# shadimsaleh/motion_detection

Hardware: AMD Instinct MI355X
Metric: Mpixels/s (flow+warp+diff) at 1080p & 4K; % HBM roofline, 1/2/4/8 GPU (higher is better)
Workload: dtype u8

## Files before the change

### motion_detection_amd/csrc/mdx_ctx.h

```cpp
#pragma once

#include "../../include/mdx.h"
#include "mdx_internal.h"

#include <algorithm>
#include <array>
#include <cstdarg>
#include <cstdio>
#include <initializer_list>
#include <string>
#include <utility>
#include <vector>

struct DevBuf {
    void* p = nullptr;
    size_t cap = 0;
    DevBuf() = default;
    DevBuf(DevBuf&& o) noexcept : p(std::exchange(o.p, nullptr)), cap(std::exchange(o.cap, 0)) {}
    DevBuf& operator=(DevBuf&& o) noexcept
    {
        std::swap(p, o.p), std::swap(cap, o.cap);
        return *this;
    }
    ~DevBuf() { reset(); }
// ... 33 lines not shown
    std::vector<hipStream_t> streams;
    std::vector<hipEvent_t> events;
    std::vector<void*> pinned;
    hipStream_t stream = nullptr;
    hipStream_t aux = nullptr;
    hipEvent_t lkev[mdx::kMaxLevels + 2] = {};
    hipStream_t iter2 = nullptr;
    hipEvent_t flowev[2] = {};
    hipEvent_t front_ev = nullptr;
    hipEvent_t pyr_free[2] = {};
    hipEvent_t lvl_done[mdx::kMaxLevels] = {};
    hipEvent_t redo_ev[mdx::kMaxLevels] = {};
    mdx::LkLaunch lk;
    int pyr_half = 0;
    hipEvent_t input_ev = nullptr;
    uint8_t* last_pyr1 = nullptr;
    uint8_t* last_pyr2 = nullptr;
    uint8_t* band_pyr1 = nullptr;
    uint8_t* band_pyr2 = nullptr;
    int band_half = 0;
    const uint8_t* band_img1 = nullptr;
    int band_built[2] = {0, 0};
    int band_stride = 0, band_fmt = 0;
    DevBuf errw;
    int* err_host = nullptr;
    int* tcnt_host = nullptr;
    long long lk_fallback[3] = {0, 0, 0};
    mdx_params prm{};
    int max_w = 0, max_h = 0, max_batch = 0;
    DevBuf pyr1, pyr2, der, fits;
    DevBuf in1, in2, np, st, vec, mask, H, Hext, num;
    DevBuf bnp, bst;
    DevBuf cls, Abuf, ctab;
    DevBuf dbg;
    DevBuf lkcnt;
    DevBuf csum;
    DevBuf tin, tcur, tnp, tst, ttraj, tnum, tflag;
    DevBuf straj, sdata, sq, scnt, scols, sres, sout, sbest;
    DevBuf clpts, clbest, clroot;
    std::vector<int32_t> cl_host;
    DevBuf vcpts, vcroot, vcrows, vcq;
    std::vector<double> vc_host;
    std::vector<float> vc_pts;
    std::vector<int32_t> vc_idx;
    DevBuf hlin, hlout;
    std::vector<int32_t> hl_in, hl_out;
    std::vector<int32_t> hl_idx;
    DevBuf olin, olmag, olout;
    std::vector<double> ol_host;
    std::vector<uint8_t> ol_flags;
    DevBuf rgscr;
    DevBuf rgin, rgout;
    DevBuf rhscr;
    DevBuf rhout;
    DevBuf ring_pyr, ring_der, rin;
    DevBuf rfull;
    DevBuf hsrc, hdst;
    DevBuf wscr;
    mdx::WarpLaunch last_warp;
    DevBuf rsc;
    std::vector<int> ring_order;
    int ring_cap = 0, ring_w = 0, ring_h = 0, ring_ml = -1;
    std::array<size_t, 4> lk_scratch_key{{0, 0, 0, 0}};
    std::array<int, 6> plan_key{{-1, -1, -1, -1, -1, -1}};
    int band_w = 0, band_h = 0;
    mdx::ClassPlan plan{};
// ... 118 lines not shown
```

### motion_detection_amd/csrc/mdx_internal.h

```cpp
#pragma once

#include <hip/hip_runtime.h>
#include <math.h>
#include <stdint.h>

#include <algorithm>

#include "mdx.h"
#include "mdx_plan.h"

namespace mdx {

static_assert(sizeof(float4) == kFloat4Bytes, "lk_scratch sizes the A sums by it");
constexpr int kLkDbgStampOff = kMaxLevels * 64 + 64;
constexpr int kLkDbgWaves = 16384;

inline uint8_t* level0_core(uint8_t* slab, const Geometry& g) { return slab + g.lv[0].img_off + g.lv[0].core(); }

struct PairFit {
    double H[9];
    double Hinv[9];
    int num_vectors;
    int fit_status;
    int src_y0, src_y1;
// ... 74 lines not shown
    int* num;
    double mvs;
    float* htraj;
    int* htlen;
    float* hstart;
    double* hvec;
};
hipError_t launch_lk_chain(hipStream_t s, const LkArgs& a, const TrajChain& t, int ppw);
size_t subspace_basis_bytes(int n, int d, int precision);
hipError_t launch_subspace(hipStream_t s, const float* traj, int N, int T, int d, const int* cols, int nhyp,
                           double sigma, float* data, void* basis, int* counts, double* residuals,
                           uint8_t* is_outlier, int* best, int precision);
constexpr int kClB = 256;
hipError_t launch_cluster(hipStream_t s, const float* pts, int N, uint32_t slim, unsigned long long* best,
                          int32_t* root);
size_t vcluster_rows_bytes(int nA);
hipError_t launch_vcluster(hipStream_t s, const double* xyt, int nA, double slim, double athr, int abs_int,
                           uint32_t* rows, uint32_t* qscan, uint32_t* cand, int32_t* root);
hipError_t launch_outliers(hipStream_t s, int batch, int n, const double* dxy, double* ang, double* mag,
                           int include_zeros, uint8_t* flags, mdx_outlier_stats* stats, bool in_registers);
hipError_t launch_traj_init(hipStream_t s, int npts, int ny, int pixel_step, int nimg, float* cur, float* traj,
                            int* tlen, int* num, int* flag = nullptr);
hipError_t launch_traj_update(hipStream_t s, int npts, const float* next_pts, const uint8_t* status, float* cur,
                              float* traj, int* tlen, int nimg, int w, int h, int last, double min_vector_size,
                              double* vectors, float* start_pts, int* num);
struct LkLaunch {
    hipStream_t s = nullptr;
    hipStream_t aux = nullptr;
    hipStream_t s2 = nullptr;
    hipEvent_t* ev = nullptr;
    hipEvent_t* flow_ev = nullptr;
    hipEvent_t* redo_ev = nullptr;
    uint8_t* cls = nullptr;
    float4* Ab = nullptr;
    uint8_t* cert = nullptr;
    int* qctr = nullptr;
    int* done = nullptr;
    hipEvent_t* lvl_done = nullptr;
    hipEvent_t prev_ready = nullptr;
};
hipError_t launch_lk_v2(const LkLaunch& L, int batch, const LkArgs& a);
constexpr int kRansacMaxIters = 1024;
struct RansacArgs {
    int iters;
    double thresh;
    uint32_t seed;
    int* list;
    double* hyps;
    int* counts;
};
struct RansacScratch {
    size_t hyps, counts, bytes;
};
inline RansacScratch ransac_scratch(int batch, int npts, int iters)
{
    const size_t list_b = (size_t)batch * npts * sizeof(int), hyps_b = (size_t)batch * iters * 9 * sizeof(double),
                 counts_b = (size_t)batch * iters * sizeof(int);
    RansacScratch L;
    L.hyps = (list_b + 7) & ~(size_t)7;
    L.counts = L.hyps + hyps_b;
    L.bytes = list_b + hyps_b + counts_b + 256;
    return L;
}
inline size_t ransac_scratch_bytes(int batch, int npts, int iters) { return ransac_scratch(batch, npts, iters).bytes; }
inline RansacArgs ransac_args(void* base, int batch, int npts, const mdx_params& P)
{
// ... 108 lines not shown
```

### motion_detection_amd/csrc/mdx_lk.hip

```cpp
#include "mdx_dev.h"

#include <float.h>

#include <algorithm>
#include <atomic>
#include <cstdlib>
#include <type_traits>

namespace mdx {

typedef short s2 __attribute__((ext_vector_type(2)));
typedef float f2 __attribute__((ext_vector_type(2)));
typedef unsigned int v4u __attribute__((ext_vector_type(4)));
typedef unsigned int v3u __attribute__((ext_vector_type(3)));
struct LkRunRsrc {
    unsigned long long base;
    uint32_t bytes;

    __device__ __forceinline__ LkRunRsrc(const void* p, uint32_t n)
    {
        const unsigned long long b = (unsigned long long)(uintptr_t)p;
        const uint32_t lo = __builtin_amdgcn_readfirstlane((uint32_t)b);
        const uint32_t hi = __builtin_amdgcn_readfirstlane((uint32_t)(b >> 32)) & 0xffffu;
        base = ((unsigned long long)hi << 32) | lo;
// ... 86 lines not shown
__device__ __forceinline__ void lk_vmcnt()
{
    static_assert(N >= 0 && N < 16, "vmcnt field");
    __builtin_amdgcn_sched_barrier(0);
    __builtin_amdgcn_s_waitcnt(0x0F70 | N);
    __builtin_amdgcn_sched_barrier(0);
}

template <int B, int E, typename F>
__device__ __forceinline__ void static_for(F&& f)
{
    if constexpr (B < E) {
        f(std::integral_constant<int, B>{});
        static_for<B + 1, E>(f);
    }
}

__device__ __forceinline__ int xcd_remap(int b, int total)
{
    const int xcd = b & 7, q = total >> 3, r = total & 7;
    return (xcd < r ? xcd * (q + 1) : r * (q + 1) + (xcd - r) * q) + (b >> 3);
}

__device__ __forceinline__ void cls_store(uint4* o, const uint32_t (&dv)[4], const int (&cv)[4])
{
    typedef unsigned v4nt __attribute__((ext_vector_type(4)));
    const uint4 a = make_uint4(dv[0], (uint32_t)cv[0], dv[1], (uint32_t)cv[1]);
    const uint4 b = make_uint4(dv[2], (uint32_t)cv[2], dv[3], (uint32_t)cv[3]);
    __builtin_nontemporal_store(__builtin_bit_cast(v4nt, a), reinterpret_cast<v4nt*>(o));
    __builtin_nontemporal_store(__builtin_bit_cast(v4nt, b), reinterpret_cast<v4nt*>(o) + 1);
}

__global__ __launch_bounds__(256) void k_lk_class(const uint8_t* __restrict__ pyr1, const uint32_t* __restrict__ der,
                                                  uint8_t* __restrict__ cls_out, LkClassArgs a)
{
    const int level = a.level;
    const ClassLevel& C = a.plan.lv[level];
    const int nclass = C.nrx * C.nry;
    const int pair = blockIdx.z / nclass, cls = blockIdx.z % nclass;
    const int j = blockIdx.x * blockDim.x + threadIdx.x;
    const int v = C.vlo + blockIdx.y;
    if (4 * j >= a.g.lv[level].w + 2 * kPad || v >= C.UH) return;
    const Level L = a.g.lv[level];
    const float scale = (float)(1. / (1 << level));
    const int rx = residue_of(a.rlist, level, 0, cls % C.nrx), ry = residue_of(a.rlist, level, 1, cls / C.nrx);
    const float ppx = (float)rx * scale - 19.5f, ppy = (float)ry * scale - 19.5f;
    const float fa = ppx - floorf(ppx), fb = ppy - floorf(ppy);
    int w00, w01, w10, w11;
    lk_weights(fa, fb, w00, w01, w10, w11);
    const uint8_t* I = pyr1 + (long long)pair * a.g.img_bytes + L.img_off + L.core();
    const uint32_t* D = der + (long long)pair * a.g.der_words + L.der_off + L.core();
    const int y = v - kPad;
    const int p = L.pitch;
    uint8_t* base = cls_out + (long long)pair * a.plan.bytes_per_pair + C.off + (long long)cls * C.class_bytes;
    uint32_t dv[4] = {0, 0, 0, 0};
    int cv[4];
    const int x0 = 4 * j - kPad;
    if (y < L.h + kPad - 1 && x0 < L.w + kPad - 1) {
        const uint8_t* ip = I + (long long)y * p + x0;
        const uint32_t* dp = D + (long long)y * p + x0;
        uint32_t ib[2][2], dw[2][5];
#pragma unroll
        for (int r = 0; r < 2; r++) {
            const u2a4k bi = *reinterpret_cast<const u2a4k*>(ip + (long long)r * p);
            ib[r][0] = bi.x; ib[r][1] = bi.y;
            const uint4 d4 = *reinterpret_cast<const uint4*>(dp + (long long)r * p);
            dw[r][0] = d4.x; dw[r][1] = d4.y; dw[r][2] = d4.z; dw[r][3] = d4.w;
            dw[r][4] = dp[(long long)r * p + 4];
        }
        const s2 W0 = {(short)w00, (short)w01}, W1 = {(short)w10, (short)w11};
        static_for<0, 4>([&](auto qc) {
            constexpr int q = decltype(qc)::value;
            if (x0 + q >= L.w + kPad - 1) { cv[q] = lk_class_c(0); return; }
            int ival, ixv, iyv;
            lk_interp<q>(ib[0][0], ib[0][1], ib[1][0], ib[1][1], dw[0][q], dw[0][q + 1], dw[1][q], dw[1][q + 1], W0, W1,
                         ival, ixv, iyv);
            dv[q] = ((uint32_t)ixv & 0xffffu) | ((uint32_t)iyv << 16);
            cv[q] = lk_class_c(ival);
        });
    } else {
#pragma unroll
        for (int q = 0; q < 4; q++) cv[q] = lk_class_c(0);
    }
    uint4* o = reinterpret_cast<uint4*>(base) + ((long long)v * C.PW + 4 * j) / 2;
    cls_store(o, dv, cv);
}

__global__ __launch_bounds__(256) void k_lk_class_fused(const uint8_t* __restrict__ pyr1, uint8_t* __restrict__ cls_out,
                                                        LkClassArgs a)
{
    const int level = a.level;
    const ClassLevel& C = a.plan.lv[level];
    const int nclass = C.nrx * C.nry;
    const int pair = blockIdx.z;
    const int j = blockIdx.x * blockDim.x + threadIdx.x;
    const int v = C.vlo + blockIdx.y;
    if (4 * j >= a.g.lv[level].w + 2 * kPad || v >= C.UH) return;
    const Level L = a.g.lv[level];
    const float scale = (float)(1. / (1 << level));
    const uint8_t* I = pyr1 + (long long)pair * a.g.img_bytes + L.img_off + L.core();
    const int y = v - kPad;
    const int p = L.pitch;
    const int x0 = 4 * j - kPad;
    const bool inside = y < L.h + kPad - 1 && x0 < L.w + kPad - 1;
    uint32_t rw[4][3];
#pragma unroll
    for (int r = 0; r < 4; r++) {
        const int yy = y - 1 + r;
        const int ys = (yy < -kPad || yy >= L.h + kPad) ? y : yy;
        const u3a4k t = *reinterpret_cast<const u3a4k*>(I + (long long)ys * p + x0 - 4);
        rw[r][0] = t.x; rw[r][1] = t.y; rw[r][2] = t.z;
    }
    uint32_t dw[2][5];
#pragma unroll
    for (int r = 0; r < 2; r++) {
        const int yy = y + r;
#pragma unroll
        for (int c = 0; c < 5; c++) {
            const int x = x0 + c;
            const bool in = yy >= 0 && yy < L.h && x >= 0 && x < L.w;
            dw[r][c] = in ? scharr_word(rw[r], rw[r + 1], rw[r + 2], 4 + c) : 0u;
        }
    }
    for (int cls = 0; cls < nclass; cls++) {
        const int rx = residue_of(a.rlist, level, 0, cls % C.nrx), ry = residue_of(a.rlist, level, 1, cls / C.nrx);
        const float ppx = (float)rx * scale - 19.5f, ppy = (float)ry * scale - 19.5f;
        const float fa = ppx - floorf(ppx), fb = ppy - floorf(ppy);
        int w00, w01, w10, w11;
        lk_weights(fa, fb, w00, w01, w10, w11);
        uint32_t dv[4] = {0, 0, 0, 0};
        int cv[4] = {lk_class_c(0), lk_class_c(0), lk_class_c(0), lk_class_c(0)};
        if (inside) {
            const s2 W0 = {(short)w00, (short)w01}, W1 = {(short)w10, (short)w11};
            static_for<0, 4>([&](auto qc) {
                constexpr int q = decltype(qc)::value;
                if (x0 + q >= L.w + kPad - 1) return;
                int ival, ixv, iyv;
                lk_interp<q>(rw[1][1], rw[1][2], rw[2][1], rw[2][2], dw[0][q], dw[0][q + 1], dw[1][q], dw[1][q + 1], W0,
                             W1, ival, ixv, iyv);
                dv[q] = ((uint32_t)ixv & 0xffffu) | ((uint32_t)iyv << 16);
                cv[q] = lk_class_c(ival);
            });
        }
        uint8_t* base = cls_out + (long long)pair * a.plan.bytes_per_pair + C.off + (long long)cls * C.class_bytes;
        uint4* o = reinterpret_cast<uint4*>(base) + ((long long)v * C.PW + 4 * j) / 2;
        cls_store(o, dv, cv);
    }
}

template <int G, int UW>
struct LkShape {
    static constexpr int UWIDTH = UW;
    static constexpr int LPS = 4 * G;
    static constexpr int S = 64 / LPS;
    static constexpr int NP = (UW + 2 * LPS - 1) / (2 * LPS);
    static constexpr int BYTES = S * UW * 8;
    static constexpr int ND = (BYTES + 1023) / 1024;
    static_assert(UW % 2 == 0 && UW >= kWin, "union width");
};

struct GroupGeom {
    int gx, gy;
    bool valid;
    int ipx, ipy;
    int off;
    int v0;
    uint32_t ubase;
};

template <int G, int UW>
__device__ __forceinline__ GroupGeom group_geom(const LkArgs& a, const ClassLevel& C, int level, int g, int sl)
{
    GroupGeom r;
    const int16_t* xo = a.ord + C.ord_off;
    const int16_t* yo = xo + C.nxp;
    const bool has = g >= 0;
    const int gg = has ? g : 0;
    const int cg = gg / a.nyg, row = gg - cg * a.nyg;
    const int e0 = cg * G;
// ... 44 lines not shown
#pragma unroll
        for (int c = 0; c < Sh::ND; c++)
            if (1024 * c + 16 * lane >= Sh::BYTES) uoff[c] = 0x80000000u;
    }
    template <int B>
    __device__ __forceinline__ void dma(const uint32_t (&uoff)[Sh::ND])
    {
        lds_u32* I = ibuf<B>();
        const __amdgpu_buffer_rsrc_t r = crs.rsrc();
#pragma unroll
        for (int c = 0; c < Sh::ND; c++)
            __builtin_amdgcn_raw_ptr_buffer_load_lds(r, (lds_ptr)(I + 256 * c), 16, (int)uoff[c], 0, 0, 0);
        crs.advance(rowb);
    }
};

__device__ __forceinline__ float4 lk_A_result(f2 sd, float s12, bool ok, float min_eig)
{
    constexpr float FLT_SCALE = 1.f / (1 << 20);
    const float a11 = ((quad_bcast<0>(sd.x) + quad_bcast<1>(sd.x)) + quad_bcast<2>(sd.x)) + quad_bcast<3>(sd.x);
    const float a12 = ((quad_bcast<0>(s12) + quad_bcast<1>(s12)) + quad_bcast<2>(s12)) + quad_bcast<3>(s12);
    const float a22 = ((quad_bcast<0>(sd.y) + quad_bcast<1>(sd.y)) + quad_bcast<2>(sd.y)) + quad_bcast<3>(sd.y);
    const float A11 = a11 * FLT_SCALE, A12 = a12 * FLT_SCALE, A22 = a22 * FLT_SCALE;
    float Dinv = 0.f;
    if (ok) {
        const float D = A11 * A22 - A12 * A12;
        const float minEig = (A22 + A11 - __builtin_sqrtf((A11 - A22) * (A11 - A22) + 4.f * A12 * A12)) /
                             (float)(2 * kWin * kWin);
        if (!(minEig < min_eig || D < FLT_EPSILON)) Dinv = 1.f / D;
    }
    return make_float4(A11, A12, A22, Dinv);
}

constexpr float kLkCertMax = 2056.f;
static_assert(kLkCertMax * 8160.f < 16777216.f, "certified products are exact in float");
__device__ __forceinline__ float lk_mag_max(float m, f2 f)
{
    return __builtin_fmaxf(__builtin_fmaxf(m, __builtin_fabsf(f.x)), __builtin_fabsf(f.y));
}
__device__ __forceinline__ f2 lk_fma(f2 f, float fd, f2 acc) { return __builtin_elementwise_fma(f, f2{fd, fd}, acc); }
__device__ __forceinline__ uint8_t lk_cert_flag(float m)
{
    const float q = __builtin_fmaxf(__builtin_fmaxf(quad_bcast<0>(m), quad_bcast<1>(m)),
                                    __builtin_fmaxf(quad_bcast<2>(m), quad_bcast<3>(m)));
    return q <= kLkCertMax ? 1 : 0;
}

template <int G, int UW>
__global__ __launch_bounds__(64) void k_lk_A(LkArgs a, const uint8_t* __restrict__ cls, float4* __restrict__ Ab,
                                             uint8_t* __restrict__ cert, int* __restrict__ qctr, int level, int ngroups)
{
    using Sh = LkShape<G, UW>;
    constexpr int LPS = Sh::LPS, S = Sh::S, ND = Sh::ND;
    constexpr int NB = 3;
    __shared__ __attribute__((aligned(16))) uint32_t img0[ND * 256];
    __shared__ __attribute__((aligned(16))) uint32_t img1[ND * 256];
    __shared__ __attribute__((aligned(16))) uint32_t img2[ND * 256];

    const int lane = threadIdx.x, k = lane & 3, slot = lane / LPS, sl = lane % LPS;
    const int nw = gridDim.x;
    const int bid = xcd_remap(blockIdx.x + nw * blockIdx.y, nw * gridDim.y);
    const int pair = bid / nw, w = bid % nw;
    if (bid == 0 && lane < 8) qctr[(level * 8 + lane) * kCtrPad] = 0;
    const ClassLevel& C = a.plan.lv[level];
    const Level L = a.g.lv[level];
    const int g = w * S + slot;
    const GroupGeom q = group_geom<G, UW>(a, C, level, g < ngroups ? g : -1, sl);
    bool ok = q.valid && !(q.ipx < -kWin || q.ipx >= L.w || q.ipy < -kWin || q.ipy >= L.h);

    LkRowImages<Sh> im{(lds_u32*)img0, (lds_u32*)img1, (lds_u32*)img2,
                       LkRunRsrc(cls + (long long)pair * a.plan.bytes_per_pair,
                                 (uint32_t)min(a.plan.bytes_per_pair, (long long)0x7fffffff)),
                       (uint32_t)C.PW * 8};
    uint32_t uoff[ND];
    lk_piece_offsets<Sh>(q.ubase + (uint32_t)q.v0 * im.rowb, lane, uoff);
    im.mask_past(lane, uoff);
    const int el = 2 * (slot * UW + q.off + k);

// ... 135 lines not shown
            nextj++;
        }
        const unsigned short ri = (unsigned short)(uint32_t)rmag;
#pragma unroll
        for (int s = 0; s < NW / 2; s++) magp[s] = __builtin_elementwise_max(magp[s], us2{ri, ri});
        static_for<0, NW>([&](auto sc) {
            constexpr int s = decltype(sc)::value;
            if (rin[s] >= 0) {
#pragma unroll
                for (int gi = 0; gi < 10; gi++) {
                    sd[s] = __builtin_elementwise_fma(f[gi], f[gi], sd[s]);
                    s12[s] = __builtin_fmaf(f[gi].x, f[gi].y, s12[s]);
                }
                if (++rin[s] == kWin) {
                    finish(jw[s], sd[s], s12[s], (float)magp[s / 2][s & 1]);
                    rin[s] = -1;
                }
            }
        });
    };
    im.template dma<0>(uoff);
    if (R > 1) im.template dma<1>(uoff);
#pragma unroll 1
    for (int t = 0; t < R; t += 3) {
        row(t, std::integral_constant<int, 0>{});
        if (t + 1 < R) row(t + 1, std::integral_constant<int, 1>{});
        if (t + 2 < R) row(t + 2, std::integral_constant<int, 2>{});
    }
}

template <int G, int UW, bool DF>
__global__ __launch_bounds__(64) __attribute__((amdgpu_waves_per_eu(kLkIterWavesPerEU, 8))) void k_lk_iter(
    LkArgs a, const uint8_t* __restrict__ cls, const float4* __restrict__ Ab, const uint8_t* __restrict__ cert,
    int* __restrict__ qctr, int level, int ngroups, int batch)
{
    using Sh = LkShape<G, UW>;
    constexpr int LPS = Sh::LPS, S = Sh::S, ND = Sh::ND;
    constexpr float HALFW = 19.5f;
    constexpr float JD_UNSCALE = 1.f / kLkJScale;
    constexpr float FLT_SCALE = 1.f / (1 << 20) * JD_UNSCALE;
    static_assert(FLT_SCALE == 1.f / (1 << 29), "2^-20 * 2^-9");
    constexpr int UB = S * UW;
    static_assert(kWin % 2 == 0, "row schedule (row pairs)");
    constexpr bool WHOLE = 2 * ND * 1024 + 2 * 1024 <= 6656;
    constexpr int UWORDS = WHOLE ? ND * 256 : 2 * UB;
    static_assert(UWORDS >= 2 * UB, "the buffer covers the union image");
    __shared__ __attribute__((aligned(16))) uint32_t dU0[UWORDS];
    __shared__ __attribute__((aligned(16))) uint32_t dU1[UWORDS];
    __shared__ __attribute__((aligned(16))) uint32_t dJ0[256];
    __shared__ __attribute__((aligned(16))) uint32_t dJ1[256];

    const int lane = threadIdx.x, k = lane & 3, slot = lane / LPS, sl = lane % LPS;
    const unsigned long long smask = ((1ull << LPS) - 1) << (slot * LPS);
    const unsigned long long t_start = a.dbg ? __builtin_amdgcn_s_memrealtime() : 0ull;
    const int xcd = blockIdx.x & 7;
    int* const a_done = DF ? a.done : nullptr;
    int* const a_lflags = DF ? a.lflags : nullptr;
    const int a_redo = DF ? a.redo : 0;
    const int dep_groups = DF ? a.dep_groups : 0;
    const long long T = (long long)batch * ngroups;
    const long long cb = T * xcd / 8, ce = T * (xcd + 1) / 8;
    const int p0 = (int)(cb / ngroups);
    const uint32_t off0 = (uint32_t)(cb - (long long)p0 * ngroups);
    const int np = ce > cb ? (int)((ce - 1) / ngroups) - p0 + 1 : 1;
    int* ctr = qctr + (level * 8 + xcd) * kCtrPad;
    if (a_redo) {
        int need = __hip_atomic_load(a_lflags + (kLkFlagGiveup + level) * kCtrPad, __ATOMIC_RELAXED,
// ... 139 lines not shown
                    if (!live) retire();
                }
            }
        }
        if (!__any(live)) break;

        f2 acc = {0.f, 0.f};
        if (act) iters++;
        int inx = (int)floorf(nx), iny = (int)floorf(ny);
        if (act && (inx < -kWin || inx >= L.w || iny < -kWin || iny >= L.h)) {
            act = false;
            if (level == 0) status = 0;
        }
        if (!act) { inx = 0; iny = 0; }
        const float fa = nx - (float)inx, fb = ny - (float)iny;
        int v00, v01, v10, v11;
        lk_weights(fa, fb, v00, v01, v10, v11);
        const s2 W0 = {(short)v00, (short)v01};
        const s2 W1 = {(short)v10, (short)v11};
        const int o = (inx & 3) + k;
        const unsigned sel = (unsigned)o | 0x0c00u | ((unsigned)(o + 1) << 16) | 0x0c000000u;
        const uint32_t joff = k < 3 ? jrel + jbase + (uint32_t)(iny * pitch + (inx & ~3) + 16 * k) : kNoFetch;
        uint32_t uoff[ND];
        lk_piece_offsets<Sh>(q.ubase + (uint32_t)q.v0 * rowb, lane, uoff);
        if (WHOLE && 1024 * (ND - 1) + 16 * lane >= Sh::BYTES) uoff[ND - 1] = kNoFetch;
        auto ubuf = [&](auto bc) -> uint32_t* {
            if constexpr (decltype(bc)::value == 0) return dU0;
            else return dU1;
        };
        auto jbuf = [&](auto bc) -> uint32_t* {
            if constexpr (decltype(bc)::value == 0) return dJ0;
            else return dJ1;
        };
        LkRunRsrc ur(cls_base, cls_bytes), jr(j_base, j_bytes);
        auto dma_union = [&](auto bc) {
            uint32_t* U = ubuf(bc);
            const __amdgpu_buffer_rsrc_t r = ur.rsrc();
#pragma unroll
            for (int c = 0; c < ND; c++) {
                if (WHOLE || c < ND - 1 || 1024 * c + 16 * lane < Sh::BYTES)
                    __builtin_amdgcn_raw_ptr_buffer_load_lds(r, (lds_ptr)(U + 256 * c), 16, (int)uoff[c], 0, 0, 0);
            }
            ur.advance(rowb);
        };
        auto dma_j = [&](auto bc) {
            __builtin_amdgcn_raw_ptr_buffer_load_lds(jr.rsrc(), (lds_ptr)jbuf(bc), 16, (int)joff, 0, 0, 0);
            jr.advance((uint32_t)pitch);
        };
        const int jl = (lane >> 2) * 16, el = 2 * (slot * UW + q.off + k);
        auto read_j = [&](auto bc, uint32_t (&rj)[11]) {
            lds_u4v* lJ = (lds_u4v*)(jbuf(bc) + jl);
            const v4u j0 = lJ[0], j1 = lJ[1], j2 = lJ[2];
            rj[0] = j0.x; rj[1] = j0.y; rj[2] = j0.z; rj[3] = j0.w;
            rj[4] = j1.x; rj[5] = j1.y; rj[6] = j1.z; rj[7] = j1.w;
            rj[8] = j2.x; rj[9] = j2.y; rj[10] = j2.z;
        };
        using I0 = std::integral_constant<int, 0>;
        using I1 = std::integral_constant<int, 1>;
        s2 pa[10], pb[10];
        dma_union(I0{});
        dma_j(I0{});
        dma_j(I1{});
        lk_vmcnt0();
        {
            uint32_t rj[11];
            read_j(I0{}, rj);
#pragma unroll
            for (int gi = 0; gi < 10; gi++) pa[gi] = __builtin_bit_cast(s2, __builtin_amdgcn_perm(rj[gi + 1], rj[gi], sel));
        }
        auto row = [&](auto Fc, int y, auto Rc, s2 (&up)[10], s2 (&lo)[10]) {
            constexpr bool FUSED = decltype(Fc)::value;
            constexpr int R = decltype(Rc)::value;
            if (y + 1 < kWin) dma_union(std::integral_constant<int, 1 - R>{});
            if (y + 2 <= kWin) dma_j(Rc);
            __builtin_amdgcn_sched_barrier(0);
            uint32_t rj[11];
            read_j(std::integral_constant<int, 1 - R>{}, rj);
            lds_u2v* lE = (lds_u2v*)(ubuf(Rc) + el);
            v2u dcs[10];
#pragma unroll
            for (int gi = 0; gi < 10; gi++) dcs[gi] = lE[4 * gi];
#pragma unroll
            for (int gi = 0; gi < 10; gi++) {
                const v2u dc = dcs[gi];
                lo[gi] = __builtin_bit_cast(s2, __builtin_amdgcn_perm(rj[gi + 1], rj[gi], sel));
                const float fd = lk_jd512((uint32_t)__builtin_amdgcn_sdot2(
                    up[gi], W0, __builtin_amdgcn_sdot2(lo[gi], W1, (int)dc.y, false), false));
                const f2 f = {(float)(int16_t)dc.x, (float)((int)dc.x >> 16)};
                if constexpr (FUSED) acc = lk_fma(f, fd, acc);
                else acc = acc + f * fd;
            }
            asm volatile("" : "+v"(acc));
            lk_vmcnt0();
        };
        const bool fused = a.fma && __all(!act || certd);
        if (a.body_cnt) (fused ? n_fused : n_exact)++;
        auto rows = [&](auto Fc) {
#pragma unroll 1
            for (int y = 0; y < kWin; y += 2) {
                row(Fc, y, I0{}, pa, pb);
                row(Fc, y + 1, I1{}, pb, pa);
            }
        };
        if (fused) rows(std::true_type{});
        else rows(std::false_type{});
        if (!act) acc = f2{0.f, 0.f};
        const float b1s = (quad_bcast<0>(acc.x) + quad_bcast<2>(acc.x)) + (quad_bcast<1>(acc.x) + quad_bcast<3>(acc.x));
        const float b2s = (quad_bcast<0>(acc.y) + quad_bcast<2>(acc.y)) + (quad_bcast<1>(acc.y) + quad_bcast<3>(acc.y));
        if (act) {
            const float b1 = b1s * FLT_SCALE, b2 = b2s * FLT_SCALE;
            const float dx = (A12 * b2 - A22 * b1) * Dinv;
            const float dy = (A12 * b1 - A11 * b2) * Dinv;
            if (a.dbg && pt == a.dbg_pt && pair == 0) {
                float4* t = a.dbg + (long long)a.g.nlev * a.npts + (level * 16 + j) * 4;
                const f2 tacc = acc * JD_UNSCALE;
                if (k == 0) {
                    t[0] = make_float4(b1s * JD_UNSCALE, b2s * JD_UNSCALE, dx, dy);
                    t[1] = make_float4(nx, ny, A11, Dinv);
                }
                t[2 + (k >> 1)] = make_float4(k & 1 ? 0.f : tacc.x, k & 1 ? 0.f : tacc.y, tacc.x, tacc.y);
            }
            nx = nx + dx;
            ny = ny + dy;
            npx = nx + HALFW;
            npy = ny + HALFW;
            if ((double)dx * dx + (double)dy * dy <= a.eps2) {
                act = false;
            } else if (j > 0 && fabs((double)fabsf(dx + pdx)) < 0.01 && fabs((double)fabsf(dy + pdy)) < 0.01) {
                npx = npx - dx * 0.5f;
// ... 66 lines not shown
        v = std::max(1, ncu) * std::max(1, nb);
        if (dev >= 0 && dev < kDevs) cached[dev].store(v, std::memory_order_relaxed);
    }
    return v;
}

static int lk_groups(const ClassPlan& plan, int l, int nyg) { return (plan.lv[l].nxp / plan.lv[l].G) * nyg; }

template <int G, int UW>
static void launch_A(hipStream_t s, int batch, const LkArgs& a, const uint8_t* cls, float4* Ab, uint8_t* cert, int* qctr,
                     int l)
{
    constexpr int S = LkShape<G, UW>::S;
    const int ngroups = lk_groups(a.plan, l, a.nyg);
    const dim3 grid((ngroups + S - 1) / S, batch);
    hipLaunchKernelGGL((k_lk_A<G, UW>), grid, dim3(64), 0, s, a, cls, Ab, cert, qctr, l, ngroups);
}

template <int G, int UW>
static void launch_A_rows(hipStream_t s, int batch, const LkArgs& a, const uint8_t* cls, float4* Ab, uint8_t* cert,
                          int* qctr, int l)
{
    constexpr int S = LkShape<G, UW>::S;
    const ClassLevel& C = a.plan.lv[l];
    const int ncg = C.nxp / G;
    const dim3 grid(((ncg + S - 1) / S) * C.nstrip, batch);
    if (C.asp >= 10)
        hipLaunchKernelGGL((k_lk_A_rows<G, UW, 4>), grid, dim3(64), 0, s, a, cls, Ab, cert, qctr, l, ncg);
    else
        hipLaunchKernelGGL((k_lk_A_rows<G, UW, 8>), grid, dim3(64), 0, s, a, cls, Ab, cert, qctr, l, ncg);
}

template <int G, int UW>
static void launch_iter(hipStream_t s, int batch, const LkArgs& a, const uint8_t* cls, const float4* Ab,
                        const uint8_t* cert, int* qctr, int l)
{
    constexpr int S = LkShape<G, UW>::S;
    const int ngroups = lk_groups(a.plan, l, a.nyg);
    const int need = (int)std::min<long long>(((long long)batch * ngroups + S - 1) / S, 1 << 30);
    const bool df = a.done || a.redo || a.lflags || a.dep_groups;
    int res = df ? lk_iter_resident<G, UW, true>() : lk_iter_resident<G, UW, false>();
    if (a.done) res = res * std::min(std::max(a.flow_cap, 10), 100) / 100;
    int W = std::max(8, std::min((need + 7) / 8, res / 8) * 8);
    if (a.redo) W = std::max(8, std::min(W, kLkRedoWaves));
    if (df)
        hipLaunchKernelGGL((k_lk_iter<G, UW, true>), dim3(W), dim3(64), 0, s, a, cls, Ab, cert, qctr, l, ngroups, batch);
    else
        hipLaunchKernelGGL((k_lk_iter<G, UW, false>), dim3(W), dim3(64), 0, s, a, cls, Ab, cert, qctr, l, ngroups, batch);
}

static bool launch_level(bool iter, hipStream_t st, int batch, const LkArgs& a, const uint8_t* cls, float4* Ab,
                         uint8_t* cert, int* qctr, int l)
{
    const ClassLevel& C = a.plan.lv[l];
    switch (C.G * 1000 + C.UW) {
#define LK_CASE(g, uw)                                                   \
    case g * 1000 + uw:                                                  \
        if (iter) launch_iter<g, uw>(st, batch, a, cls, Ab, cert, qctr, l);    \
        else if (C.asp) launch_A_rows<g, uw>(st, batch, a, cls, Ab, cert, qctr, l); \
        else launch_A<g, uw>(st, batch, a, cls, Ab, cert, qctr, l);            \
        return true;
        LK_SHAPES
#undef LK_CASE
    default: return false;
    }
}

static hipError_t lk_enqueue_planes(const LkLaunch& L, hipStream_t sa, int batch, int p, int nb, const LkArgs& a,
                                    const LkArgs& b, uint8_t* bcls, int* bq)
{
    if (L.aux) {
        hipEvent_t ready = L.prev_ready;
        if (!ready || p) {
            if (hipError_t e = hipEventRecord(L.ev[kMaxLevels], L.s)) return e;
            ready = L.ev[kMaxLevels];
        }
        if (hipError_t e = hipStreamWaitEvent(sa, ready, 0)) return e;
    }
    for (int l = a.maxl; l >= 0; l--) {
        const ClassLevel& C = a.plan.lv[l];
        if (L.aux && L.lvl_done) {
            if (hipError_t e = hipStreamWaitEvent(sa, L.lvl_done[l], 0)) return e;
        }
        LkClassArgs ca;
        ca.g = a.g;
        ca.plan = a.plan;
        ca.rlist = a.rlist;
        ca.level = l;
        if (C.nrx * C.nry <= 4) {
            const dim3 grid(((a.g.lv[l].w + 2 * kPad) / 4 + 63) / 64, C.vhi - C.vlo, nb);
            hipLaunchKernelGGL(k_lk_class_fused, grid, dim3(64), 0, sa, b.pyr1, bcls, ca);
        } else {
            const dim3 grid(((a.g.lv[l].w + 2 * kPad) / 4 + 63) / 64, C.vhi - C.vlo, nb * C.nrx * C.nry);
            if (hipError_t e = launch_scharr(sa, nb, b.pyr1, const_cast<uint32_t*>(b.der), a.g, l, C.vlo, C.vhi + 1))
                return e;
            hipLaunchKernelGGL(k_lk_class, grid, dim3(64), 0, sa, b.pyr1, b.der, bcls, ca);
        }
        float4* bA = L.Ab + ((long long)l * batch + p) * a.npts;
        uint8_t* bC = L.cert + ((long long)l * batch + p) * a.npts;
        if (!launch_level(false, sa, nb, b, bcls, bA, bC, bq, l)) return hipErrorInvalidValue;
        if (L.aux) {
            if (hipError_t e = hipEventRecord(L.ev[l], sa)) return e;
        }
    }
    return hipSuccess;
}

static hipError_t lk_enqueue_iters(const LkLaunch& L, int batch, int p, int nb, const LkArgs& a, const LkArgs& b,
                                   uint8_t* bcls, int* bq)
{
    const bool flow_ok = L.aux && L.s2 && L.flow_ev && L.done && L.redo_ev && a.err && b.carry &&
                         (reinterpret_cast<uintptr_t>(b.carry) & 127) == 0 && (a.carry_lstride % 32) == 0;
    const bool flow = flow_ok && nb % 8 == 0 && nb >= 16 && a.npts % 16 == 0 &&
                      (reinterpret_cast<uintptr_t>(b.next_pts) & 127) == 0;
    int* lflags = flow ? L.done + (long long)kMaxLevels * nb * kCtrPad : nullptr;
    if (flow) {
        if (hipError_t e = hipMemsetAsync(L.done, 0, sizeof(int) * ((long long)kMaxLevels * nb + kLkFlagInts) * kCtrPad, L.s))
            return e;
        if (hipError_t e = hipEventRecord(L.flow_ev[0], L.s)) return e;
        if (hipError_t e = hipStreamWaitEvent(L.s2, L.flow_ev[0], 0)) return e;
    }
    for (int l = a.maxl; l >= 0; l--) {
        hipStream_t st = flow && ((a.maxl - l) & 1) ? L.s2 : L.s;
        if (L.aux) {
            if (hipError_t e = hipStreamWaitEvent(st, L.ev[l], 0)) return e;
        }
        LkArgs bl = b;
        bl.done = flow ? L.done : nullptr;
        bl.done_stride = nb;
        bl.dep_groups = 0;
        bl.lflags = lflags;
        bl.redo = 0;
        if (flow && l < a.maxl) {
            const int ngc = lk_groups(a.plan, l + 1, a.nyg), ng = lk_groups(a.plan, l, a.nyg);
            bl.dep_groups = ngc;
            hipLaunchKernelGGL(k_lk_gate, dim3(1), dim3(64), 0, st, bq + (l + 1) * 8 * kCtrPad, (long long)nb * ngc,
                               L.done + (l + 1) * nb * kCtrPad, bl.dep_groups, ng, (long long)nb * ng, a.err,
                               a.spin_max, lflags + (kLkFlagGiveup + l) * kCtrPad);
        }
        float4* bA = L.Ab + ((long long)l * batch + p) * a.npts;
        uint8_t* bC = L.cert + ((long long)l * batch + p) * a.npts;
        if (!launch_level(true, st, nb, bl, bcls, bA, bC, bq, l)) return hipErrorInvalidValue;
        if (flow) {
            if (l < a.maxl) {
                if (hipError_t e = hipStreamWaitEvent(st, L.redo_ev[l + 1], 0)) return e;
                LkArgs br = bl;
                br.done = nullptr;
                br.dep_groups = 0;
                br.redo = 1;
                br.dbg = nullptr;
                br.body_cnt = nullptr;
                if (!launch_level(true, st, nb, br, bcls, bA, bC, bq, l)) return hipErrorInvalidValue;
            }
            if (hipError_t e = hipEventRecord(L.redo_ev[l], st)) return e;
        }
        if (L.lvl_done) {
            if (hipError_t e = hipEventRecord(L.lvl_done[l], st)) return e;
        }
    }
    if (flow) {
        if (hipError_t e = hipEventRecord(L.flow_ev[1], L.s2)) return e;
        if (hipError_t e = hipStreamWaitEvent(L.s, L.flow_ev[1], 0)) return e;
    }
    return hipSuccess;
}

hipError_t launch_lk_v2(const LkLaunch& L, int batch, const LkArgs& a)
{
    const long long span = std::max(a.plan.bytes_per_pair, a.g.img_bytes);
    int sub = batch;
    while (sub > 1 && ((sub + 7) / 8 + 1) * span > 0x7fff0000LL) sub = std::max(1, sub / 2);
    if (a.max_sub > 0) sub = std::max(1, std::min(sub, a.max_sub));
    hipStream_t sa = L.aux ? L.aux : L.s;
    for (int p = 0, si = 0; p < batch; p += sub, si++) {
        const int nb = std::min(sub, batch - p);
        LkArgs b = a;
        b.pyr1 = a.pyr1 + (long long)p * a.g.img_bytes;
        b.pyr2 = a.pyr2 + (long long)p * a.g.img_bytes;
        b.der = a.der + (long long)p * a.g.der_words;
        b.next_pts = a.next_pts + (long long)p * a.npts * 2;
        b.carry = a.carry ? a.carry + (long long)p * a.npts * 2 : nullptr;
        b.status = a.status + (long long)p * a.npts;
        if (p) b.dbg = nullptr;
        uint8_t* bcls = L.cls + (long long)p * a.plan.bytes_per_pair;
        int* bq = L.qctr + si * kMaxLevels * 8 * kCtrPad;
        if (hipError_t e = lk_enqueue_planes(L, sa, batch, p, nb, a, b, bcls, bq)) return e;
        if (hipError_t e = lk_enqueue_iters(L, batch, p, nb, a, b, bcls, bq)) return e;
    }
    return hipGetLastError();
}

}
```

### motion_detection_amd/csrc/mdx_pair.cpp

```cpp
#include "mdx_ctx.h"

#include <cmath>
#include <cstdlib>
#include <new>

using namespace mdx;

static int ensure_class_plan(mdx_ctx* c, const Geometry& g, int w, int h, int ps, int batch, int gy0, int gy1)
{
    int rc;
    const std::array<int, 6> key = {w, h, ps, g.nlev, gy0, gy1};
    if (c->plan_key != key) {
        BuiltPlan B;
        try {
            B = build_class_plan(g, w, h, ps, gy0, gy1, PlanTuning{c->lk_g, c->lk_astrip, c->max_batch});
        } catch (const std::bad_alloc&) {
            return set_err(c, MDX_ENOMEM, "class plan: out of host memory");
        }
        if ((rc = ensure(c, c->ctab, B.tab.size() * sizeof(int16_t))) != MDX_OK) return rc;
        HIP_OR_RETURN(c, hipStreamSynchronize(c->stream));
        HIP_OR_RETURN(c, hipMemcpy(c->ctab.p, B.tab.data(), B.tab.size() * sizeof(int16_t), hipMemcpyHostToDevice));
        c->plan = B.plan;
        c->plan_key = key;
    }
    if (c->plan.nch == 0) return MDX_OK;
    return ensure(c, c->cls, (size_t)c->plan.bytes_per_pair * batch + 64);
}

static int wait_input(mdx_ctx* c, hipStream_t st)
{
    if (!c->input_ev) return MDX_OK;
    hipEvent_t e = c->input_ev;
    c->input_ev = nullptr;
    HIP_OR_RETURN(c, hipStreamWaitEvent(st, e, 0));
    return MDX_OK;
}

int mdx::run_lk(mdx_ctx* c, const Geometry& g, LkArgs& a, int batch, int w, int h, int gy0, int gy1, bool have_scharr,
                hipEvent_t prev_ready)
{
    int rc;
    hipStream_t s = c->stream;
    bool v2 = c->lk_impl == 2 && a.prev_pts == nullptr;
    if (v2) {
        if ((rc = ensure_class_plan(c, g, w, h, c->prm.pixel_step, batch, gy0, gy1)) != MDX_OK) return rc;
        v2 = c->plan.nch != 0;
    }
    if (!v2) {
        if (gy0 != 0 || gy1 != a.ny)
            return set_err(c, MDX_EINVAL, "row bands need the class-plane LK (pixel_step too large)");
        if (!have_scharr) HIP_OR_RETURN(c, launch_scharr_levels(s, batch, a.pyr1, const_cast<uint32_t*>(a.der), g));
        HIP_OR_RETURN(c, launch_lk(s, batch, a));
        return MDX_OK;
    }
    a.plan = c->plan;
    a.max_sub = c->lk_sub;
    a.err = c->errw.as<int>();
    a.spin_max = c->spin_max;
    a.flow_cap = c->lk_cap;
    a.fma = c->lk_fma ? 1 : 0;
    a.cmap = c->ctab.as<int16_t>();
    a.rlist = c->ctab.as<int16_t>() + kTabRlist;
    a.ord = c->ctab.as<int16_t>() + kTabOrd;
    const int npts = a.npts;
    if (c->lk_debug) {
        if ((rc = ensure(c, c->dbg, ((size_t)npts * g.nlev * batch + kLkDbgStampOff + kMaxLevels * kLkDbgWaves) * 16)) !=
            MDX_OK)
            return rc;
        a.dbg = c->dbg.as<float4>();
        const char* e = std::getenv("MDX_LK_DEBUG_PT");
        a.dbg_pt = e ? std::atoi(e) : -1;
        if ((rc = ensure(c, c->lkcnt, kMaxLevels * 2 * sizeof(uint32_t))) != MDX_OK) return rc;
        HIP_OR_RETURN(c, hipMemsetAsync(c->lkcnt.p, 0, kMaxLevels * 2 * sizeof(uint32_t), s));
        a.body_cnt = c->lkcnt.as<uint32_t>();
    }
    const LkScratch sc = lk_scratch(g.nlev, batch, npts);
    if ((rc = ensure(c, c->Abuf, sc.bytes)) != MDX_OK) return rc;
    const std::array<size_t, 4> lay = {reinterpret_cast<size_t>(c->Abuf.p), (size_t)g.nlev, (size_t)batch, (size_t)npts};
    if (c->lk_scratch_key != lay) {
        HIP_OR_RETURN(c, hipStreamSynchronize(c->stream));
        c->lk_scratch_key = lay;
    }
    uint8_t* base = c->Abuf.as<uint8_t>();
    a.carry = reinterpret_cast<float*>(base + sc.carry);
    a.carry_lstride = (long long)(sc.carry_level / sizeof(float));
    LkLaunch L = c->lk;
    L.cls = c->cls.as<uint8_t>();
    L.Ab = c->Abuf.as<float4>();
    L.cert = base + sc.cert;
    L.qctr = reinterpret_cast<int*>(base + sc.qctr);
    L.done = reinterpret_cast<int*>(base + sc.done);
    L.lvl_done = c->prm.call_pipelining ? c->lvl_done : nullptr;
    L.prev_ready = prev_ready;
    HIP_OR_RETURN(c, launch_lk_v2(L, batch, a));
    return MDX_OK;
}

static int run_warp_diff(mdx_ctx* c, int batch, const WarpArgs& a)
{
    const size_t wsb = warp_scratch_bytes(batch, a.w, (a.row1 < 0 ? a.h : a.row1) - a.row0);
    if (const int rc = ensure(c, c->wscr, wsb); rc != MDX_OK) return rc;
    HIP_OR_RETURN(c, launch_warp_diff(c->stream, batch, a, c->wscr.p, wsb, &c->last_warp));
    return MDX_OK;
}
static GrayPlane pyr_gray(uint8_t* slab, const Geometry& g)
{
    return {level0_core(slab, g), g.img_bytes, g.lv[0].pitch};
}

struct PipelineArgs {
    int batch;
    const uint8_t *d_img1, *d_img2;
    int w, h, stride;
    size_t frame_stride;
    int fmt;
    float* d_np;
    uint8_t* d_st;
    double* d_vec = nullptr;
    uint8_t* d_mask = nullptr;
    double* d_H = nullptr;
// ... 273 lines not shown
```

### motion_detection_amd/csrc/mdx_plan.h

```cpp
#pragma once

#include <math.h>
#include <stddef.h>
#include <stdint.h>

#include <algorithm>
#include <vector>

#ifdef __HIPCC__
#define MDX_HD __host__ __device__
#else
#define MDX_HD
#endif

namespace mdx {

constexpr int kMaxLevels = 8;
constexpr int kWin = 40;
constexpr int kPad = 40;
constexpr int kXOff = 64;

struct Level {
    int w, h;
    int pitch;
// ... 49 lines not shown
    int asp;
    int nstrip;
    int strip_off;
};
constexpr int kAStripRows = 16;

MDX_HD inline int lk_win_origin(int gi, int pixel_step, int level)
{
    return (int)floorf((float)(gi * pixel_step) * (float)(1. / (1 << level)) - 19.5f);
}
MDX_HD inline int lk_win_row0(int ipy, int UH) { return std::min(std::max(ipy + kPad, 0), UH - kWin); }

constexpr uint32_t kLkJBiasWord = 0x4B400000u;
constexpr float kLkJBiasFloat = 12582912.f;
constexpr uint32_t kLkJMask = 0xFFFFFE00u;
constexpr int kLkJScale = 512;
constexpr int kLkJShift = 9;
constexpr int kLkSMin = -255, kLkSMax = 16385 * 255;
constexpr int kLkIMax = 8160;
constexpr int kLkXMin = kLkSMin + 256 - 512 * kLkIMax, kLkXMax = kLkSMax + 256;
static_assert(16385 * 255 + 256 < (1 << 22), "largest x stays inside the mantissa field's upper half");
static_assert(512 * 8160 + 255 - 256 < (1 << 22), "smallest x stays inside its lower half");
static_assert((kLkJBiasWord & 0x7FFFFFu) == (1u << 22), "the bias puts x = 0 in the middle of the mantissa field");
static_assert(kLkJBiasWord >> 23 == 127 + 23, "exponent 2^23: one mantissa step is 1");
static_assert((1 << kLkJShift) == kLkJScale && kLkJMask == ~(uint32_t)(kLkJScale - 1), "mask, shift and scale agree");
constexpr int kLkCBias = (int)kLkJBiasWord + 256;
MDX_HD inline int lk_class_c(int ival) { return kLkCBias - 512 * ival; }
MDX_HD inline float lk_jd512(uint32_t biased)
{
    const uint32_t w = biased & kLkJMask;
    float f;
    __builtin_memcpy(&f, &w, sizeof(f));
    return f - kLkJBiasFloat;
}

#define LK_SHAPES LK_CASE(4, 48) LK_CASE(4, 56) LK_CASE(4, 64) LK_CASE(4, 72) LK_CASE(4, 80) LK_CASE(4, 96) \
    LK_CASE(4, 128) LK_CASE(8, 80) LK_CASE(8, 112) LK_CASE(8, 128) LK_CASE(8, 256) LK_CASE(8, 512)
constexpr int kLkUW4[] = {48, 56, 64, 72, 80, 96, 128};
constexpr int kLkUW8[] = {80, 112, 128, 256, 512};

struct ClassPlan {
    ClassLevel lv[kMaxLevels];
    long long bytes_per_pair;
    int nch;
};

constexpr int kCtrPad = 32;
constexpr int kLkFlagGiveup = 0;
constexpr int kLkFlagRedone = kMaxLevels;
constexpr int kLkFlagQueue = 2 * kMaxLevels;
constexpr int kLkFlagInts = kLkFlagQueue + 8 * kMaxLevels;

struct RowSpan {
    int lo, hi;
};

constexpr int kTabStride = 128;
static_assert(kMaxLevels <= 8, "residue tables sized for 2^7 residues");
constexpr int kTabRlist = kMaxLevels * 2 * kTabStride;
constexpr int kTabOrd = 2 * kTabRlist;

struct PlanTuning {
    int lk_g;
    int lk_astrip;
    int max_batch;
};
// ... 195 lines not shown
```

Measured before the change: 9448.

## Store derivatives as packed fp16 copy and use fma_mix in certified LK path

The class kernels now also write a second class plane holding the gradient pair as packed half floats. The certified fused LK iteration reads this plane and uses v_fma_mix_f32 to accumulate directly from the halves, which removes the int16 unpack and convert per element. The certification bound drops from 2056 to 2048 so the halves stay exact. The cost is a second class buffer, double store traffic in the class kernels, and slightly fewer points taking the fused path.

```diff
diff --git a/motion_detection_amd/csrc/mdx_ctx.h b/motion_detection_amd/csrc/mdx_ctx.h
--- a/motion_detection_amd/csrc/mdx_ctx.h
+++ b/motion_detection_amd/csrc/mdx_ctx.h
@@ -89,6 +89,7 @@
     DevBuf in1, in2, np, st, vec, mask, H, Hext, num;
     DevBuf bnp, bst;
     DevBuf cls, Abuf, ctab;
+    DevBuf cls_h;
     DevBuf dbg;
     DevBuf lkcnt;
     DevBuf csum;
diff --git a/motion_detection_amd/csrc/mdx_internal.h b/motion_detection_amd/csrc/mdx_internal.h
--- a/motion_detection_amd/csrc/mdx_internal.h
+++ b/motion_detection_amd/csrc/mdx_internal.h
@@ -130,6 +130,7 @@
     hipEvent_t* flow_ev = nullptr;
     hipEvent_t* redo_ev = nullptr;
     uint8_t* cls = nullptr;
+    uint8_t* cls_h = nullptr;
     float4* Ab = nullptr;
     uint8_t* cert = nullptr;
     int* qctr = nullptr;
diff --git a/motion_detection_amd/csrc/mdx_lk.hip b/motion_detection_amd/csrc/mdx_lk.hip
--- a/motion_detection_amd/csrc/mdx_lk.hip
+++ b/motion_detection_amd/csrc/mdx_lk.hip
@@ -142,7 +142,8 @@
 }
 
 __global__ __launch_bounds__(256) void k_lk_class(const uint8_t* __restrict__ pyr1, const uint32_t* __restrict__ der,
-                                                  uint8_t* __restrict__ cls_out, LkClassArgs a)
+                                                  uint8_t* __restrict__ cls_out, uint8_t* __restrict__ clsh_out,
+                                                  LkClassArgs a)
 {
     const int level = a.level;
     const ClassLevel& C = a.plan.lv[level];
@@ -162,8 +163,8 @@
     const uint32_t* D = der + (long long)pair * a.g.der_words + L.der_off + L.core();
     const int y = v - kPad;
     const int p = L.pitch;
-    uint8_t* base = cls_out + (long long)pair * a.plan.bytes_per_pair + C.off + (long long)cls * C.class_bytes;
-    uint32_t dv[4] = {0, 0, 0, 0};
+    const long long cbase = (long long)pair * a.plan.bytes_per_pair + C.off + (long long)cls * C.class_bytes;
+    uint32_t dv[4] = {0, 0, 0, 0}, hv[4] = {0, 0, 0, 0};
     int cv[4];
     const int x0 = 4 * j - kPad;
     if (y < L.h + kPad - 1 && x0 < L.w + kPad - 1) {
@@ -186,18 +187,20 @@
             lk_interp<q>(ib[0][0], ib[0][1], ib[1][0], ib[1][1], dw[0][q], dw[0][q + 1], dw[1][q], dw[1][q + 1], W0, W1,
                          ival, ixv, iyv);
             dv[q] = ((uint32_t)ixv & 0xffffu) | ((uint32_t)iyv << 16);
+            hv[q] = lk_half_pair(ixv, iyv);
             cv[q] = lk_class_c(ival);
         });
     } else {
 #pragma unroll
         for (int q = 0; q < 4; q++) cv[q] = lk_class_c(0);
     }
-    uint4* o = reinterpret_cast<uint4*>(base) + ((long long)v * C.PW + 4 * j) / 2;
-    cls_store(o, dv, cv);
+    const long long eo = ((long long)v * C.PW + 4 * j) / 2;
+    cls_store(reinterpret_cast<uint4*>(cls_out + cbase) + eo, dv, cv);
+    cls_store(reinterpret_cast<uint4*>(clsh_out + cbase) + eo, hv, cv);
 }
 
 __global__ __launch_bounds__(256) void k_lk_class_fused(const uint8_t* __restrict__ pyr1, uint8_t* __restrict__ cls_out,
-                                                        LkClassArgs a)
+                                                        uint8_t* __restrict__ clsh_out, LkClassArgs a)
 {
     const int level = a.level;
     const ClassLevel& C = a.plan.lv[level];
@@ -238,7 +241,7 @@
         const float fa = ppx - floorf(ppx), fb = ppy - floorf(ppy);
         int w00, w01, w10, w11;
         lk_weights(fa, fb, w00, w01, w10, w11);
-        uint32_t dv[4] = {0, 0, 0, 0};
+        uint32_t dv[4] = {0, 0, 0, 0}, hv[4] = {0, 0, 0, 0};
         int cv[4] = {lk_class_c(0), lk_class_c(0), lk_class_c(0), lk_class_c(0)};
         if (inside) {
             const s2 W0 = {(short)w00, (short)w01}, W1 = {(short)w10, (short)w11};
@@ -249,12 +252,14 @@
                 lk_interp<q>(rw[1][1], rw[1][2], rw[2][1], rw[2][2], dw[0][q], dw[0][q + 1], dw[1][q], dw[1][q + 1], W0,
                              W1, ival, ixv, iyv);
                 dv[q] = ((uint32_t)ixv & 0xffffu) | ((uint32_t)iyv << 16);
+                hv[q] = lk_half_pair(ixv, iyv);
                 cv[q] = lk_class_c(ival);
             });
         }
-        uint8_t* base = cls_out + (long long)pair * a.plan.bytes_per_pair + C.off + (long long)cls * C.class_bytes;
-        uint4* o = reinterpret_cast<uint4*>(base) + ((long long)v * C.PW + 4 * j) / 2;
-        cls_store(o, dv, cv);
+        const long long cbase = (long long)pair * a.plan.bytes_per_pair + C.off + (long long)cls * C.class_bytes;
+        const long long eo = ((long long)v * C.PW + 4 * j) / 2;
+        cls_store(reinterpret_cast<uint4*>(cls_out + cbase) + eo, dv, cv);
+        cls_store(reinterpret_cast<uint4*>(clsh_out + cbase) + eo, hv, cv);
     }
 }
 
@@ -365,18 +370,22 @@
     return make_float4(A11, A12, A22, Dinv);
 }
 
-constexpr float kLkCertMax = 2056.f;
-static_assert(kLkCertMax * 8160.f < 16777216.f, "certified products are exact in float");
 __device__ __forceinline__ float lk_mag_max(float m, f2 f)
 {
     return __builtin_fmaxf(__builtin_fmaxf(m, __builtin_fabsf(f.x)), __builtin_fabsf(f.y));
 }
-__device__ __forceinline__ f2 lk_fma(f2 f, float fd, f2 acc) { return __builtin_elementwise_fma(f, f2{fd, fd}, acc); }
+__device__ __forceinline__ f2 lk_fma_half(uint32_t hd, float fd, f2 acc)
+{
+    float x = acc.x, y = acc.y;
+    asm("v_fma_mix_f32 %0, %1, %2, %0 op_sel_hi:[0,1,0]" : "+v"(x) : "v"(fd), "v"(hd));
+    asm("v_fma_mix_f32 %0, %1, %2, %0 op_sel:[0,1,0] op_sel_hi:[0,1,0]" : "+v"(y) : "v"(fd), "v"(hd));
+    return f2{x, y};
+}
 __device__ __forceinline__ uint8_t lk_cert_flag(float m)
 {
     const float q = __builtin_fmaxf(__builtin_fmaxf(quad_bcast<0>(m), quad_bcast<1>(m)),
                                     __builtin_fmaxf(quad_bcast<2>(m), quad_bcast<3>(m)));
-    return q <= kLkCertMax ? 1 : 0;
+    return q <= (float)kLkCertMax ? 1 : 0;
 }
 
 template <int G, int UW>
@@ -578,7 +587,7 @@
 template <int G, int UW, bool DF>
 __global__ __launch_bounds__(64) __attribute__((amdgpu_waves_per_eu(kLkIterWavesPerEU, 8))) void k_lk_iter(
     LkArgs a, const uint8_t* __restrict__ cls, const float4* __restrict__ Ab, const uint8_t* __restrict__ cert,
-    int* __restrict__ qctr, int level, int ngroups, int batch)
+    int* __restrict__ qctr, int level, int ngroups, int batch, const uint8_t* __restrict__ clsh)
 {
     using Sh = LkShape<G, UW>;
     constexpr int LPS = Sh::LPS, S = Sh::S, ND = Sh::ND;
@@ -784,7 +793,9 @@
             if constexpr (decltype(bc)::value == 0) return dJ0;
             else return dJ1;
         };
-        LkRunRsrc ur(cls_base, cls_bytes), jr(j_base, j_bytes);
+        const bool fused = a.fma && __all(!act || certd);
+        if (a.body_cnt) (fused ? n_fused : n_exact)++;
+        LkRunRsrc ur(fused ? clsh + (long long)p0 * a.plan.bytes_per_pair : cls_base, cls_bytes), jr(j_base, j_bytes);
         auto dma_union = [&](auto bc) {
             uint32_t* U = ubuf(bc);
             const __amdgpu_buffer_rsrc_t r = ur.rsrc();
@@ -838,15 +849,16 @@
                 lo[gi] = __builtin_bit_cast(s2, __builtin_amdgcn_perm(rj[gi + 1], rj[gi], sel));
                 const float fd = lk_jd512((uint32_t)__builtin_amdgcn_sdot2(
                     up[gi], W0, __builtin_amdgcn_sdot2(lo[gi], W1, (int)dc.y, false), false));
-                const f2 f = {(float)(int16_t)dc.x, (float)((int)dc.x >> 16)};
-                if constexpr (FUSED) acc = lk_fma(f, fd, acc);
-                else acc = acc + f * fd;
+                if constexpr (FUSED) {
+                    acc = lk_fma_half(dc.x, fd, acc);
+                } else {
+                    const f2 f = {(float)(int16_t)dc.x, (float)((int)dc.x >> 16)};
+                    acc = acc + f * fd;
+                }
             }
             asm volatile("" : "+v"(acc));
             lk_vmcnt0();
         };
-        const bool fused = a.fma && __all(!act || certd);
-        if (a.body_cnt) (fused ? n_fused : n_exact)++;
         auto rows = [&](auto Fc) {
 #pragma unroll 1
             for (int y = 0; y < kWin; y += 2) {
@@ -979,8 +991,8 @@
 }
 
 template <int G, int UW>
-static void launch_iter(hipStream_t s, int batch, const LkArgs& a, const uint8_t* cls, const float4* Ab,
-                        const uint8_t* cert, int* qctr, int l)
+static void launch_iter(hipStream_t s, int batch, const LkArgs& a, const uint8_t* cls, const uint8_t* clsh,
+                        const float4* Ab, const uint8_t* cert, int* qctr, int l)
 {
     constexpr int S = LkShape<G, UW>::S;
     const int ngroups = lk_groups(a.plan, l, a.nyg);
@@ -991,19 +1003,19 @@
     int W = std::max(8, std::min((need + 7) / 8, res / 8) * 8);
     if (a.redo) W = std::max(8, std::min(W, kLkRedoWaves));
     if (df)
-        hipLaunchKernelGGL((k_lk_iter<G, UW, true>), dim3(W), dim3(64), 0, s, a, cls, Ab, cert, qctr, l, ngroups, batch);
+        hipLaunchKernelGGL((k_lk_iter<G, UW, true>), dim3(W), dim3(64), 0, s, a, cls, Ab, cert, qctr, l, ngroups, batch, clsh);
     else
-        hipLaunchKernelGGL((k_lk_iter<G, UW, false>), dim3(W), dim3(64), 0, s, a, cls, Ab, cert, qctr, l, ngroups, batch);
-}
-
-static bool launch_level(bool iter, hipStream_t st, int batch, const LkArgs& a, const uint8_t* cls, float4* Ab,
-                         uint8_t* cert, int* qctr, int l)
+        hipLaunchKernelGGL((k_lk_iter<G, UW, false>), dim3(W), dim3(64), 0, s, a, cls, Ab, cert, qctr, l, ngroups, batch, clsh);
+}
+
+static bool launch_level(bool iter, hipStream_t st, int batch, const LkArgs& a, const uint8_t* cls, const uint8_t* clsh,
+                         float4* Ab, uint8_t* cert, int* qctr, int l)
 {
     const ClassLevel& C = a.plan.lv[l];
     switch (C.G * 1000 + C.UW) {
 #define LK_CASE(g, uw)                                                   \
     case g * 1000 + uw:                                                  \
-        if (iter) launch_iter<g, uw>(st, batch, a, cls, Ab, cert, qctr, l);    \
+        if (iter) launch_iter<g, uw>(st, batch, a, cls, clsh, Ab, cert, qctr, l); \
         else if (C.asp) launch_A_rows<g, uw>(st, batch, a, cls, Ab, cert, qctr, l); \
         else launch_A<g, uw>(st, batch, a, cls, Ab, cert, qctr, l);            \
         return true;
@@ -1014,7 +1026,7 @@
 }
 
 static hipError_t lk_enqueue_planes(const LkLaunch& L, hipStream_t sa, int batch, int p, int nb, const LkArgs& a,
-                                    const LkArgs& b, uint8_t* bcls, int* bq)
+                                    const LkArgs& b, uint8_t* bcls, uint8_t* bclsh, int* bq)
 {
     if (L.aux) {
         hipEvent_t ready = L.prev_ready;
@@ -1036,16 +1048,16 @@
         ca.level = l;
         if (C.nrx * C.nry <= 4) {
             const dim3 grid(((a.g.lv[l].w + 2 * kPad) / 4 + 63) / 64, C.vhi - C.vlo, nb);
-            hipLaunchKernelGGL(k_lk_class_fused, grid, dim3(64), 0, sa, b.pyr1, bcls, ca);
+            hipLaunchKernelGGL(k_lk_class_fused, grid, dim3(64), 0, sa, b.pyr1, bcls, bclsh, ca);
         } else {
             const dim3 grid(((a.g.lv[l].w + 2 * kPad) / 4 + 63) / 64, C.vhi - C.vlo, nb * C.nrx * C.nry);
             if (hipError_t e = launch_scharr(sa, nb, b.pyr1, const_cast<uint32_t*>(b.der), a.g, l, C.vlo, C.vhi + 1))
                 return e;
-            hipLaunchKernelGGL(k_lk_class, grid, dim3(64), 0, sa, b.pyr1, b.der, bcls, ca);
+            hipLaunchKernelGGL(k_lk_class, grid, dim3(64), 0, sa, b.pyr1, b.der, bcls, bclsh, ca);
         }
         float4* bA = L.Ab + ((long long)l * batch + p) * a.npts;
         uint8_t* bC = L.cert + ((long long)l * batch + p) * a.npts;
-        if (!launch_level(false, sa, nb, b, bcls, bA, bC, bq, l)) return hipErrorInvalidValue;
+        if (!launch_level(false, sa, nb, b, bcls, bclsh, bA, bC, bq, l)) return hipErrorInvalidValue;
         if (L.aux) {
             if (hipError_t e = hipEventRecord(L.ev[l], sa)) return e;
         }
@@ -1054,7 +1066,7 @@
 }
 
 static hipError_t lk_enqueue_iters(const LkLaunch& L, int batch, int p, int nb, const LkArgs& a, const LkArgs& b,
-                                   uint8_t* bcls, int* bq)
+                                   uint8_t* bcls, uint8_t* bclsh, int* bq)
 {
     const bool flow_ok = L.aux && L.s2 && L.flow_ev && L.done && L.redo_ev && a.err && b.carry &&
                          (reinterpret_cast<uintptr_t>(b.carry) & 127) == 0 && (a.carry_lstride % 32) == 0;
@@ -1087,7 +1099,7 @@
         }
         float4* bA = L.Ab + ((long long)l * batch + p) * a.npts;
         uint8_t* bC = L.cert + ((long long)l * batch + p) * a.npts;
-        if (!launch_level(true, st, nb, bl, bcls, bA, bC, bq, l)) return hipErrorInvalidValue;
+        if (!launch_level(true, st, nb, bl, bcls, bclsh, bA, bC, bq, l)) return hipErrorInvalidValue;
         if (flow) {
             if (l < a.maxl) {
                 if (hipError_t e = hipStreamWaitEvent(st, L.redo_ev[l + 1], 0)) return e;
@@ -1097,7 +1109,7 @@
                 br.redo = 1;
                 br.dbg = nullptr;
                 br.body_cnt = nullptr;
-                if (!launch_level(true, st, nb, br, bcls, bA, bC, bq, l)) return hipErrorInvalidValue;
+                if (!launch_level(true, st, nb, br, bcls, bclsh, bA, bC, bq, l)) return hipErrorInvalidValue;
             }
             if (hipError_t e = hipEventRecord(L.redo_ev[l], st)) return e;
         }
@@ -1130,9 +1142,10 @@
         b.status = a.status + (long long)p * a.npts;
         if (p) b.dbg = nullptr;
         uint8_t* bcls = L.cls + (long long)p * a.plan.bytes_per_pair;
+        uint8_t* bclsh = L.cls_h + (long long)p * a.plan.bytes_per_pair;
         int* bq = L.qctr + si * kMaxLevels * 8 * kCtrPad;
-        if (hipError_t e = lk_enqueue_planes(L, sa, batch, p, nb, a, b, bcls, bq)) return e;
-        if (hipError_t e = lk_enqueue_iters(L, batch, p, nb, a, b, bcls, bq)) return e;
+        if (hipError_t e = lk_enqueue_planes(L, sa, batch, p, nb, a, b, bcls, bclsh, bq)) return e;
+        if (hipError_t e = lk_enqueue_iters(L, batch, p, nb, a, b, bcls, bclsh, bq)) return e;
     }
     return hipGetLastError();
 }
diff --git a/motion_detection_amd/csrc/mdx_pair.cpp b/motion_detection_amd/csrc/mdx_pair.cpp
--- a/motion_detection_amd/csrc/mdx_pair.cpp
+++ b/motion_detection_amd/csrc/mdx_pair.cpp
@@ -24,7 +24,8 @@
         c->plan_key = key;
     }
     if (c->plan.nch == 0) return MDX_OK;
-    return ensure(c, c->cls, (size_t)c->plan.bytes_per_pair * batch + 64);
+    const size_t slab = (size_t)c->plan.bytes_per_pair * batch + 64;
+    return ensure_all(c, {{&c->cls, slab}, {&c->cls_h, slab}});
 }
 
 static int wait_input(mdx_ctx* c, hipStream_t st)
@@ -86,6 +87,7 @@
     a.carry_lstride = (long long)(sc.carry_level / sizeof(float));
     LkLaunch L = c->lk;
     L.cls = c->cls.as<uint8_t>();
+    L.cls_h = c->cls_h.as<uint8_t>();
     L.Ab = c->Abuf.as<float4>();
     L.cert = base + sc.cert;
     L.qctr = reinterpret_cast<int*>(base + sc.qctr);
diff --git a/motion_detection_amd/csrc/mdx_plan.h b/motion_detection_amd/csrc/mdx_plan.h
--- a/motion_detection_amd/csrc/mdx_plan.h
+++ b/motion_detection_amd/csrc/mdx_plan.h
@@ -105,6 +105,28 @@
     float f;
     __builtin_memcpy(&f, &w, sizeof(f));
     return f - kLkJBiasFloat;
+}
+
+constexpr int kLkCertMax = 2048;
+constexpr int kLkDerivMax = 4080;
+static_assert(kLkCertMax <= 2048, "binary16 holds every integer up to 2^11 exactly");
+static_assert((long long)kLkCertMax * kLkIMax < (1 << 24), "certified products are exact in float");
+MDX_HD inline uint32_t lk_half_bits(int v)
+{
+    const uint32_t s = v < 0 ? 0x8000u : 0u, m = (uint32_t)(v < 0 ? -v : v);
+    if (m == 0) return 0;
+    int e = 0;
+    while ((m >> e) > 1) e++;
+    const uint32_t frac = e <= 10 ? m << (10 - e) : m >> (e - 10);
+    return s | (uint32_t)(e + 15) << 10 | (frac & 0x3ffu);
+}
+MDX_HD inline uint32_t lk_half_pair(int ix, int iy)
+{
+#if defined(__HIP_DEVICE_COMPILE__)
+    return __builtin_bit_cast(uint32_t, __builtin_amdgcn_cvt_pkrtz((float)ix, (float)iy));
+#else
+    return lk_half_bits(ix) | lk_half_bits(iy) << 16;
+#endif
 }
 
 #define LK_SHAPES LK_CASE(4, 48) LK_CASE(4, 56) LK_CASE(4, 64) LK_CASE(4, 72) LK_CASE(4, 80) LK_CASE(4, 96) \
```

After: 9307. -1.5%, worse.
